# r-barnes/richdem

Hardware: NVIDIA H100
Metric: Priority-Flood fill + D8 flow accumulation throughput (higher is better)
Workload: dtype f32

## Files before the change

richdem_b200/csrc/accum.cu:

```cuda
#include "flowmet.cuh"

#include <cmath>
#include <cooperative_groups.h>
#include <memory>
namespace cg = cooperative_groups;

namespace rdb {

namespace {

constexpr uint32_t kDepsMask = 0xFFu;
constexpr uint32_t kSrcFlag = 0x80000000u;
constexpr int kCodeSole = 32;
constexpr int kCodeSource = 64;
constexpr int kLaneChunk = 1024;

template <bool DINF, class T = float>
__global__ void __launch_bounds__(256) flow_code_kernel(const T *__restrict__ dem, uint8_t *__restrict__ code,
                                                         float *__restrict__ rmaxArr, double *__restrict__ accum,
                                                         int W, int H, T nodata, int ones, int tfilter) {
  const size_t n = (size_t)W * H;
  const size_t i = (size_t)blockIdx.x * blockDim.x + threadIdx.x;
  if (i >= n) return;
  const int y = (int)(i / W), x = (int)(i - (size_t)y * W);
// ... 1364 lines not shown
    k = (int)(wv >> 56);
    sum[x] = (double)(wv & kPkVal);
    cnt[x] = k;
    ghost[x] = 0;
  }
  for (int o = 16; o > 0; o >>= 1) k += __shfl_down_sync(0xffffffffu, k, o);
  if ((threadIdx.x & 31) == 0 && k) atomicAdd(total, k);
}

__global__ void __launch_bounds__(256) band_count_packed_kernel(const unsigned long long *__restrict__ gtop,
                                                                 const unsigned long long *__restrict__ gbot, int W,
                                                                 int *sums) {
  int s0 = 0, s1 = 0;
  for (int x = blockIdx.x * blockDim.x + threadIdx.x; x < W; x += gridDim.x * blockDim.x) {
    if (gtop) s0 += (int)(gtop[x] >> 56);
    if (gbot) s1 += (int)(gbot[x] >> 56);
  }
  for (int o = 16; o > 0; o >>= 1) {
    s0 += __shfl_down_sync(0xffffffffu, s0, o);
    s1 += __shfl_down_sync(0xffffffffu, s1, o);
  }
  if ((threadIdx.x & 31) == 0) {
    if (s0) atomicAdd(&sums[0], s0);
    if (s1) atomicAdd(&sums[1], s1);
  }
}

__global__ void __launch_bounds__(256) band_apply_packed_kernel(unsigned long long *row, const double *__restrict__ sum,
                                                                 const int *__restrict__ cnt, int W, int base_index,
                                                                 int *frontier, int *fcount, double scale) {
  const int x = blockIdx.x * blockDim.x + threadIdx.x;
  if (x >= W) return;
  const int k = cnt[x];
  if (k <= 0) return;
  const unsigned long long wv = row[x];
  const unsigned long long val = (wv & kPkVal) + (unsigned long long)sum[x];
  const unsigned long long left = (wv >> 56) - (unsigned long long)k;
  if (left == 0) {
    row[x] = (unsigned long long)__double_as_longlong((double)val * scale);
    frontier[atomicAdd(fcount, 1)] = base_index + x;
  } else {
    row[x] = (left << 56) | val;
  }
}

constexpr int kFaT = 64;
constexpr int kFaCells = kFaT * kFaT;
constexpr int kFaSlots = 4 * kFaT;
constexpr unsigned long long kLkOne = 1ull << 32;

__device__ __forceinline__ int fa_side(int left) { return left < kFaT ? left : kFaT; }

__device__ __forceinline__ int fa_slot_of(int lx, int ly, int tw, int th) {
  if (ly == 0) return lx;
  if (ly == th - 1) return kFaT + lx;
  if (lx == 0) return 2 * kFaT + ly;
  if (lx == tw - 1) return 3 * kFaT + ly;
  return -1;
}

__device__ __forceinline__ bool fa_slot_cell(int s, int tw, int th, int &lx, int &ly) {
  const int k = s & (kFaT - 1), side = s / kFaT;
  if (side < 2) {
    lx = k;
    ly = side == 0 ? 0 : th - 1;
    return k < tw && (side == 0 || th > 1);
  }
  lx = side == 2 ? 0 : tw - 1;
  ly = k;
  return k > 0 && k < th - 1 && (side == 2 || tw > 1);
}

constexpr int kFaRootExit = 0x8000, kFaRootEnd = 0x4000, kFaRoot = kFaRootExit | kFaRootEnd;

__device__ __forceinline__ int fa_tile_parent(int c, int cd, int tw, int th) {
  const int d = cd & 15;
  if (cd == kCodeNoData || d == 0) return c | kFaRootEnd;
  const int x = (c & (kFaT - 1)) + d8dx(d), y = c / kFaT + d8dy(d);
  if (x < 0 || y < 0 || x >= tw || y >= th) return c | kFaRootExit;
  return y * kFaT + x;
}

template <bool SUM>
__device__ __forceinline__ void fa_tile_jump(uint16_t *sPar, unsigned *sAcc, unsigned live) {
  constexpr int kPer = kFaCells / 256;
  const int t = threadIdx.x;
  while (__syncthreads_or(live)) {
    unsigned pq[kPer], a[kPer];
#pragma unroll
    for (int k = 0; k < kPer; k++) {
      if (live >> k & 1) {
        const int c = t + 256 * k, p = sPar[c], q = sPar[p];
        if (SUM) {
          pq[k] = (unsigned)p | (unsigned)q << 16;
          a[k] = sAcc[c];
        } else {
          sPar[c] = (uint16_t)q;
          if (q & kFaRoot) live &= ~(1u << k);
        }
      }
    }
    if (SUM) {
      __syncthreads();
#pragma unroll
      for (int k = 0; k < kPer; k++) {
        if (live >> k & 1) {
          const int q = pq[k] >> 16;
          atomicAdd(&sAcc[pq[k] & 0xffffu], a[k]);
          sPar[t + 256 * k] = (uint16_t)q;
          if (q & kFaRoot) live &= ~(1u << k);
        }
      }
    }
  }
}

__global__ void __launch_bounds__(256) fa_tile_codes_kernel(const float *__restrict__ dem, uint8_t *__restrict__ code,
                                                             int *__restrict__ link, unsigned long long *__restrict__ lword,
                                                             unsigned *__restrict__ inflow, int W, int H, float nodata,
                                                             int tiles_x) {
  constexpr int kWin = kFaT + 2;
  static_assert(kFaCells * sizeof(uint16_t) <= kWin * kWin * sizeof(float), "the parent array lives in the DEM window");
  __shared__ __align__(16) float sDem[kWin * kWin];
  __shared__ __align__(16) uint8_t sCode[kFaCells];
  __shared__ unsigned sCount[kFaSlots];
  const int t = threadIdx.x, tile = blockIdx.x;
  sCount[t] = 0;
  const int bx = tile % tiles_x, by = tile / tiles_x;
  const int x0 = bx * kFaT, y0 = by * kFaT;
  const int tw = fa_side(W - x0), th = fa_side(H - y0);
  constexpr unsigned kFaNoDataBits = 0x7fffffffu;
  for (int i = t; i < kWin * kWin; i += 256) {
    const int wy = i / kWin, wx = i - wy * kWin;
    const int gy = y0 - 1 + wy, gx = x0 - 1 + wx;
    float v = __uint_as_float(kFaNoDataBits);
    if (gy >= 0 && gy < H && gx >= 0 && gx < W) {
      v = __ldg(dem + (size_t)gy * W + gx);
      v = v == nodata ? __uint_as_float(kFaNoDataBits) : v != v ? __uint_as_float(0x7fc00000u) : v;
    }
    sDem[i] = v;
  }
  __syncthreads();
  {
    const int lx0 = (t & 15) * 4, ly0 = (t >> 4) * 4;
    float a[3][6];
#pragma unroll
    for (int j = 1; j < 3; j++)
#pragma unroll
      for (int k = 0; k < 6; k++) a[j][k] = sDem[(ly0 + j - 1) * kWin + lx0 + k];
#pragma unroll
    for (int j = 0; j < 4; j++) {
      const int ly = ly0 + j, gy = y0 + ly;
#pragma unroll
      for (int k = 0; k < 6; k++) {
        a[0][k] = a[1][k];
        a[1][k] = a[2][k];
        a[2][k] = sDem[(ly + 2) * kWin + lx0 + k];
      }
      unsigned word = 0;
#pragma unroll
      for (int k = 0; k < 4; k++) {
        const int lx = lx0 + k, gx = x0 + lx;
        const float e = a[1][k + 1];
        int cd = 0;
        if (lx >= tw || ly >= th || __float_as_uint(e) == kFaNoDataBits) {
          cd = kCodeNoData;
        } else if (!(gx == 0 || gy == 0 || gx == W - 1 || gy == H - 1)) {
          const float ne[9] = {0.f, a[1][k], a[0][k], a[0][k + 1], a[0][k + 2], a[1][k + 2], a[2][k + 2], a[2][k + 1], a[2][k]};
          float lowest = fminf(e, 3.402823466e+38f);
#pragma unroll
          for (int n = 1; n <= 8; n++) {
            if (ne[n] < lowest) {
              lowest = ne[n];
              cd = n;
            }
          }
        }
        word |= (unsigned)cd << (8 * k);
      }
      *reinterpret_cast<unsigned *>(&sCode[ly * kFaT + lx0]) = word;
    }
  }
  __syncthreads();
  reinterpret_cast<uint4 *>(code + (size_t)tile * kFaCells)[t] = reinterpret_cast<const uint4 *>(sCode)[t];
  uint16_t *sPar = reinterpret_cast<uint16_t *>(sDem);
  unsigned live = 0;
#pragma unroll
  for (int k = 0; k < kFaCells / 256; k++) {
    const int c = t + 256 * k, p = fa_tile_parent(c, sCode[c], tw, th);
    sPar[c] = (uint16_t)p;
    if (!(p & kFaRoot)) live |= 1u << k;
  }
  fa_tile_jump<false>(sPar, nullptr, live);
#pragma unroll
  for (int k = 0; k < kFaCells / 256; k++) {
    const int r = sPar[t + 256 * k];
    if (r & kFaRootExit) atomicAdd(&sCount[fa_slot_of(r & (kFaT - 1), (r & (kFaCells - 1)) / kFaT, tw, th)], 1u);
  }
  __syncthreads();
  const size_t gs = (size_t)tile * kFaSlots + t;
  int lk = -1;
  unsigned long long out = 0;
  int lx, ly;
  if (fa_slot_cell(t, tw, th, lx, ly)) {
    const int c = ly * kFaT + lx, r = sPar[c];
    if (r == (c | kFaRootExit)) {
      const int d = sCode[c] & 15;
      const int gx = x0 + lx + d8dx(d), gy = y0 + ly + d8dy(d), rbx = gx / kFaT, rby = gy / kFaT;
      const int rs = fa_slot_of(gx - rbx * kFaT, gy - rby * kFaT, fa_side(W - rbx * kFaT), fa_side(H - rby * kFaT));
      lk = -2 - ((rby * tiles_x + rbx) * kFaSlots + rs);
      out = kLkOne | sCount[t];
    } else if (r & kFaRootExit) {
      const int e = r & (kFaCells - 1);
      lk = tile * kFaSlots + fa_slot_of(e & (kFaT - 1), e / kFaT, tw, th);
    }
  }
  link[gs] = lk;
  lword[gs] = out;
  inflow[gs] = 0;
}

__device__ __forceinline__ int fa_link_next(const int *link, int r) {
  const int l = link[r];
  return l <= -2 ? r : l;
}

__global__ void __launch_bounds__(256) fa_link_count_kernel(const int *__restrict__ link, unsigned long long *lword,
                                                             int nslots) {
  const int p = blockIdx.x * blockDim.x + threadIdx.x;
  if (p >= nslots) return;
  const int l = link[p];
  if (l > -2) return;
  const int q = fa_link_next(link, -2 - l);
  if (q >= 0) atomicAdd(&lword[q], kLkOne);
}

__global__ void __launch_bounds__(256) fa_link_walk_kernel(const int *__restrict__ link, unsigned long long *lword,
                                                            unsigned *inflow, int nslots) {
  const int p = blockIdx.x * blockDim.x + threadIdx.x;
  if (p >= nslots) return;
  int l = link[p];
  if (l > -2) return;
  const unsigned long long old = atomicAdd(&lword[p], 0ull - kLkOne);
  if ((old >> 32) != 1ull) return;
  unsigned long long acc = old & (kLkOne - 1);
  for (;;) {
    const int r = -2 - l;
    atomicAdd(&inflow[r], (unsigned)acc);
    const int q = fa_link_next(link, r);
    if (q < 0) break;
    const unsigned long long o = atomicAdd(&lword[q], acc - kLkOne);
    if ((o >> 32) != 1ull) break;
    acc = (o & (kLkOne - 1)) + acc;
    l = link[q];
  }
}

__global__ void __launch_bounds__(256) fa_tile_final_kernel(const uint8_t *__restrict__ code,
                                                             const unsigned *__restrict__ inflow, double *__restrict__ accum,
                                                             int W, int H, int tiles_x) {
  constexpr unsigned kNoDataAcc = 0xffffffffu;
  __shared__ __align__(16) unsigned sAcc[kFaCells];
  __shared__ __align__(16) uint16_t sPar[kFaCells];
  __shared__ __align__(16) uint8_t sCode[kFaCells];
  const int t = threadIdx.x, tile = blockIdx.x;
  const int bx = tile % tiles_x, by = tile / tiles_x;
  const int x0 = bx * kFaT, y0 = by * kFaT;
  const int tw = fa_side(W - x0), th = fa_side(H - y0);
  reinterpret_cast<uint4 *>(sCode)[t] = __ldg(reinterpret_cast<const uint4 *>(code + (size_t)tile * kFaCells) + t);
  __syncthreads();
  unsigned live = 0;
#pragma unroll
  for (int k = 0; k < kFaCells / 256; k++) {
    const int c = t + 256 * k, cd = sCode[c], p = fa_tile_parent(c, cd, tw, th);
    sPar[c] = (uint16_t)p;
    sAcc[c] = cd == kCodeNoData ? kNoDataAcc : 1u;
    if (!(p & kFaRoot)) live |= 1u << k;
  }
  __syncthreads();
  int lx, ly;
  if (fa_slot_cell(t, tw, th, lx, ly) && sCode[ly * kFaT + lx] != kCodeNoData)
    sAcc[ly * kFaT + lx] += __ldg(inflow + (size_t)tile * kFaSlots + t);
  fa_tile_jump<true>(sPar, sAcc, live);
  for (int c = 2 * t; c < kFaCells; c += 512) {
    const int cx = c & (kFaT - 1), cy = c / kFaT;
    if (cx >= tw || cy >= th) continue;
    const unsigned s0 = sAcc[c], s1 = sAcc[c + 1];
    const double a0 = s0 == kNoDataAcc ? -1.0 : (double)s0, a1 = s1 == kNoDataAcc ? -1.0 : (double)s1;
    double *out = accum + (size_t)(y0 + cy) * W + x0 + cx;
    if (cx + 1 < tw && ((uintptr_t)out & 15) == 0) {
      *reinterpret_cast<double2 *>(out) = make_double2(a0, a1);
    } else {
      out[0] = a0;
      if (cx + 1 < tw) out[1] = a1;
    }
  }
}

long long fa_tile_slots(int w, int h) {
  return (long long)((w + kFaT - 1) / kFaT) * ((h + kFaT - 1) / kFaT) * kFaSlots;
}

void fa_d8_tiles(const float *d_dem, double *d_accum, int w, int h, float nodata) {
  Ctx &c = ctx();
  const int tiles_x = (w + kFaT - 1) / kFaT;
  const long long nslots = fa_tile_slots(w, h);
  const unsigned ntiles = (unsigned)(nslots / kFaSlots);
  DevBuf<uint8_t> code((size_t)ntiles * kFaCells);
  DevBuf<int> link((size_t)nslots);
  DevBuf<unsigned long long> lword((size_t)nslots);
  DevBuf<unsigned> inflow((size_t)nslots);
  const unsigned sblocks = (unsigned)((nslots + 255) / 256);
  fa_tile_codes_kernel<<<ntiles, 256, 0, c.stream>>>(d_dem, code.p, link.p, lword.p, inflow.p, w, h, nodata, tiles_x);
  fa_link_count_kernel<<<sblocks, 256, 0, c.stream>>>(link.p, lword.p, (int)nslots);
  KernelTimer kt;
  fa_link_walk_kernel<<<sblocks, 256, 0, c.stream>>>(link.p, lword.p, inflow.p, (int)nslots);
  kt.stop_async();
  fa_tile_final_kernel<<<ntiles, 256, 0, c.stream>>>(code.p, inflow.p, d_accum, w, h, tiles_x);
  RDB_CK(cudaGetLastError());
  count_launch(4);
  RDB_CK(cudaStreamSynchronize(c.stream));
  c.stats.ms_main_kernel += kt.ms();
  c.stats.accum_rounds = 1;
}
}

template <class T>
static void fa_fused(const T *d_dem, double *d_accum, int w, int h, T nodata, bool ones, bool dinf) {
  constexpr bool F32 = sizeof(T) == 4;
  Ctx &c = ctx();
  const size_t n = (size_t)w * h;
  if constexpr (F32) {
    if (!dinf && ones && c.params.accum_packed && fa_tile_slots(w, h) < INT32_MAX) {
      fa_d8_tiles(d_dem, d_accum, w, h, nodata);
      return;
    }
  } else if (!dinf) {
    fail("FA_D8 on doubles runs on float keys (fa_fused_dev)");
  }
  DevBuf<uint8_t> code(n);
  DevBuf<float> rmax;
  bool have_codes = false;
  if (dinf && ones && (w & 3) == 0 && ((uintptr_t)d_accum & 15) == 0 && c.params.accum_dinf_packed) {
    rmax.alloc(n);
    const unsigned blocks = (unsigned)((n + 255) / 256);
    unsigned long long *word = reinterpret_cast<unsigned long long *>(d_accum);
    flow_code_kernel<true, T><<<blocks, 256, 0, c.stream>>>(d_dem, code.p, rmax.p, d_accum, w, h, nodata, 1, (int)c.params.flowmet_tarboton_filter);
    have_codes = true;
    DevBuf<DinfShare> share(1);
    RDB_CK(cudaMemsetAsync(share.p, 0, sizeof(DinfShare), c.stream));
    dinf_count_data_kernel<<<c.num_sms * 8, 256, 0, c.stream>>>(code.p, n, share.p);
    RDB_CK(cudaGetLastError());
    count_launch(2);
    DinfShare *hs0 = reinterpret_cast<DinfShare *>(c.pinned);
    RDB_CK(cudaMemcpyAsync(hs0, share.p, sizeof(DinfShare), cudaMemcpyDeviceToHost, c.stream));
    RDB_CK(cudaStreamSynchronize(c.stream));
    const bool use_packed = c.params.accum_dinf_packed == 1 || (long long)hs0->n_noflow * 20 > (long long)hs0->n_data;
    if (use_packed) {
    dim3 blk(256), grd((w / 4 + 255) / 256, h < 8192 ? h : 8192);
    deps_gather_packed_dinf_x4_kernel<<<grd, blk, 0, c.stream>>>(code.p, word, w, h, 0, h);
    RDB_CK(cudaGetLastError());
    count_launch();
    DevBuf<int> list(n);
    DevBuf<unsigned long long> dstats;
    if (c.params.accum_dinf_stats) {
      dstats.alloc(16);
      RDB_CK(cudaMemsetAsync(dstats.p, 0, 16 * sizeof(unsigned long long), c.stream));
    }
    KernelTimer kt;
    launch_walk_dinf(code.p, rmax.p, word, w, (int)n, list.p, share.p, dstats.p, 0, (int)n, -1);
    RDB_CK(cudaGetLastError());
    count_launch(2);
    DinfShare *hs = reinterpret_cast<DinfShare *>(c.pinned);
    RDB_CK(cudaMemcpyAsync(hs, share.p, sizeof(DinfShare), cudaMemcpyDeviceToHost, c.stream));
    kt.stop_async();
    RDB_CK(cudaStreamSynchronize(c.stream));
    c.stats.ms_main_kernel += kt.ms();
    c.stats.accum_rounds = hs->phases;
    if (dstats.p) {
      unsigned long long hsx[16];
      RDB_CK(cudaMemcpy(hsx, dstats.p, sizeof(hsx), cudaMemcpyDeviceToHost));
      fprintf(stderr,
              "[dinf walk] %.2f ms, %llu warps, %d phases: iterations sum %llu max %llu, lane-steps %llu (%.1f %% of the lanes), "
              "hand-overs %llu in the rings, %llu through the list (%llu claimed back)\n",
              kt.ms(), hsx[4], hs->phases, hsx[0], hsx[3], hsx[2], 100.0 * (double)hsx[2] / (32.0 * (double)(hsx[0] ? hsx[0] : 1)),
              hsx[8], hsx[7], hsx[6]);
    }
    if (hs->done != hs->n_data)
      fail("D-infinity accumulation (packed walk): %d of %d cells walked after %d phases", hs->done, hs->n_data, hs->phases);
    return;
    }
  }
  DevBuf<uint32_t> st(n);
  if (dinf && !have_codes) rmax.alloc(n);
  const unsigned blocks = (unsigned)((n + 255) / 256);
  if (have_codes) {
  } else if (dinf)
    flow_code_kernel<true, T><<<blocks, 256, 0, c.stream>>>(d_dem, code.p, rmax.p, d_accum, w, h, nodata, ones ? 1 : 0, (int)c.params.flowmet_tarboton_filter);
  else if constexpr (F32) {
    if ((w & 3) == 0 && ((uintptr_t)d_dem & 15) == 0 && ((uintptr_t)d_accum & 15) == 0) {
      dim3 blk(256), grd((w / 4 + 255) / 256, h < 8192 ? h : 8192);
      flow_code_d8_x4_kernel<<<grd, blk, 0, c.stream>>>(d_dem, code.p, d_accum, w, h, nodata, ones ? 1 : 0);
    } else
      flow_code_kernel<false><<<blocks, 256, 0, c.stream>>>(d_dem, code.p, nullptr, d_accum, w, h, nodata, ones ? 1 : 0, (int)c.params.flowmet_tarboton_filter);
  }
  RDB_CK(cudaGetLastError());
// ... 826 lines not shown
```

richdem_b200/csrc/capi.cu:

```cuda
#include "common.cuh"

#include <algorithm>
#include <cstdlib>
#include <type_traits>

namespace rdb {

static thread_local std::string g_last_error;

void capi_set_error(const char *msg) { g_last_error = msg ? msg : "unknown error"; }

Ctx &ctx() {
  static Ctx c;
  return c;
}

static void init_device(int device) {
  Ctx &c = ctx();
  if (c.inited && c.device == device) return;
  if (c.inited) fail("rdb200_init: already initialised on device %d (call rdb200_shutdown first)", c.device);
  int ndev = 0;
  cudaError_t e = cudaGetDeviceCount(&ndev);
  if (e != cudaSuccess || ndev == 0)
    fail("no CUDA device available (%s); librichdem_b200 has no CPU fallback",
// ... 422 lines not shown

extern "C" {

int rdb200_init(int device) {
  return capi_call([&] { init_device(device); });
}

void rdb200_shutdown(void) {
  Ctx &c = ctx();
  if (!c.inited) return;
  cudaSetDevice(c.device);
  cudaStreamSynchronize(c.stream);
  ws_release_all();
  if (c.pinned) cudaFreeHost(c.pinned);
  cudaEventDestroy(c.ev0);
  cudaEventDestroy(c.ev1);
  cudaEventDestroy(c.evk0);
  cudaEventDestroy(c.evk1);
  cudaStreamDestroy(c.own_stream);
  for (int k = 0; k < 2; k++)
    if (c.aux_stream[k]) cudaStreamDestroy(c.aux_stream[k]);
  for (int k = 0; k < 3; k++)
    if (c.aux_event[k]) cudaEventDestroy(c.aux_event[k]);
  const Params keep = c.params;
  c = Ctx();
  c.params = keep;
}

const char *rdb200_last_error(void) { return g_last_error.c_str(); }
int rdb200_version(void) { return RDB200_VERSION; }

int rdb200_set_stream(void *cuda_stream) {
  return capi_call([&] {
    ensure_init();
    Ctx &c = ctx();
    RDB_CK(cudaStreamSynchronize(c.stream));
    c.stream = cuda_stream ? (cudaStream_t)cuda_stream : c.own_stream;
  });
}

int rdb200_get_stats(rdb200_stats *out) {
  return capi_call([&] {
    if (!out) fail("rdb200_get_stats: null pointer");
    *out = ctx().stats;
  });
}

int rdb200_set_param(const char *name, int64_t value) {
  return capi_call([&] {
    if (!name) fail("rdb200_set_param: null name");
    Params &p = ctx().params;
    const std::string n(name);
    if (n == "reset_defaults") p = Params();
    else if (n == "trim_workspace") {
      if (ctx().inited) {
        RDB_CK(cudaStreamSynchronize(ctx().stream));
        ws_trim();
      }
    }
    else if (n == "fill_max_iters") p.fill_max_iters = value;
    else if (n == "fill_rounds_per_sync") p.fill_rounds_per_sync = value > 0 ? value : 16;
    else if (n == "fill_use_tma") p.fill_use_tma = value;
    else if (n == "fill_external_z") p.fill_external_z = value;
    else if (n == "fill_profile") p.fill_profile = value;
    else if (n == "fill_wake_filter") p.fill_wake_filter = value;
    else if (n == "fill_trace") p.fill_trace = value;
    else if (n == "fill_ordered") p.fill_ordered = value;
    else if (n == "fill_order_rounds") p.fill_order_rounds = value;
    else if (n == "fill_band_rounds") p.fill_band_rounds = value;
    else if (n == "accum_threads") p.accum_threads = value > 0 ? value : 256;
    else if (n == "accum_budget") p.accum_budget = value;
    else if (n == "accum_walk_lanes") p.accum_walk_lanes = value;
    else if (n == "accum_fused_prep") p.accum_fused_prep = value;
    else if (n == "flats_tiled") p.flats_tiled = value;
    else if (n == "flats_pair") p.flats_pair = value;
    else if (n == "flats_fused_classify") p.flats_fused_classify = value;
    else if (n == "fill_multigrid") p.fill_multigrid = value;
    else if (n == "fill_multigrid_min") p.fill_multigrid_min = value;
    else if (n == "fill_vcycle") p.fill_vcycle = value;
    else if (n == "fill_band_multigrid") p.fill_band_multigrid = value;
    else if (n == "flats_uf_tiled") p.flats_uf_tiled = value;
    else if (n == "flowdirs_rolling") p.flowdirs_rolling = value;
    else if (n == "accum_packed") p.accum_packed = value;
    else if (n == "accum_dinf_packed") p.accum_dinf_packed = value;
    else if (n == "accum_dinf_share") p.accum_dinf_share = value;
    else if (n == "flowmet_tarboton_filter") p.flowmet_tarboton_filter = value;
    else if (n == "accum_walk_scan") p.accum_walk_scan = value;
    else if (n == "accum_walk_ahead") p.accum_walk_ahead = value;
    else if (n == "accum_dinf_stats") p.accum_dinf_stats = value;
    else if (n == "accum_dinf_wait") p.accum_dinf_wait = value;
    else if (n == "f64_band_rank_cap") p.f64_band_rank_cap = value;
    else fail("rdb200_set_param: unknown parameter '%s'", name);
  });
}


int rdb200_fill_depressions_d8_f32(float *dem, int32_t w, int32_t h) { return fill_depressions(Side::host, dem, w, h, false); }
int rdb200_fill_depressions_d4_f32(float *dem, int32_t w, int32_t h) { return fill_depressions(Side::host, dem, w, h, true); }
int rdb200_fill_depressions_epsilon_d8_f32(float *dem, int32_t w, int32_t h, float nodata) {
  return fill_depressions_epsilon(Side::host, dem, w, h, nodata, false);
}
int rdb200_fill_depressions_epsilon_d4_f32(float *dem, int32_t w, int32_t h, float nodata) {
  return fill_depressions_epsilon(Side::host, dem, w, h, nodata, true);
}
int rdb200_pit_mask_d8_f32(const float *dem, uint8_t *mask, int32_t w, int32_t h, float nodata) {
  return pit_mask(Side::host, dem, mask, w, h, nodata, false);
}
int rdb200_pit_mask_d4_f32(const float *dem, uint8_t *mask, int32_t w, int32_t h, float nodata) {
  return pit_mask(Side::host, dem, mask, w, h, nodata, true);
}
int rdb200_has_depressions_d8_f32(const float *dem, int32_t w, int32_t h, int32_t *out) {
  return has_depressions(Side::host, dem, w, h, out, false);
}
int rdb200_has_depressions_d4_f32(const float *dem, int32_t w, int32_t h, int32_t *out) {
  return has_depressions(Side::host, dem, w, h, out, true);
}
int rdb200_resolve_flats_epsilon_f32(float *dem, int32_t w, int32_t h, float nodata) {
  return resolve_flats_epsilon(Side::host, dem, w, h, nodata);
}
int rdb200_get_flat_mask_f32(const float *dem, int32_t *flat_mask, int32_t *labels, int32_t w, int32_t h, float nodata) {
  return get_flat_mask(Side::host, dem, flat_mask, labels, w, h, nodata);
}
int rdb200_d8_flow_directions_f32(const float *dem, uint8_t *dirs, int32_t w, int32_t h, float nodata) {
  return d8_flow_directions(Side::host, dem, dirs, w, h, nodata);
}
int rdb200_d8_flow_directions_flats_f32(float *dem, uint8_t *dirs, int32_t w, int32_t h, float nodata, int32_t alter) {
  return d8_flow_directions_flats(Side::host, dem, dirs, w, h, nodata, alter);
}
int rdb200_d8_flow_accum_u8_i32(const uint8_t *dirs, int32_t *area, int32_t w, int32_t h) {
  return d8_flow_accum(Side::host, dirs, area, w, h);
}
int rdb200_fm_d8_f32(const float *dem, float *props, int32_t w, int32_t h, float nodata) {
  return fm(Side::host, 0, dem, props, w, h, nodata);
}
int rdb200_fm_tarboton_f32(const float *dem, float *props, int32_t w, int32_t h, float nodata) {
  return fm(Side::host, 1, dem, props, w, h, nodata);
}
int rdb200_fm_d4_f32(const float *dem, float *props, int32_t w, int32_t h, float nodata) {
  return fm(Side::host, 2, dem, props, w, h, nodata);
}
int rdb200_fm_quinn_f32(const float *dem, float *props, int32_t w, int32_t h, float nodata) {
  return fm(Side::host, 3, dem, props, w, h, nodata, 1.0);
}
int rdb200_fm_holmgren_f32(const float *dem, float *props, int32_t w, int32_t h, float nodata, double xparam) {
  return fm(Side::host, 3, dem, props, w, h, nodata, xparam);
}
int rdb200_fm_freeman_f32(const float *dem, float *props, int32_t w, int32_t h, float nodata, double xparam) {
  return fm(Side::host, 4, dem, props, w, h, nodata, xparam);
}
int rdb200_terrain_attribute_f32(int32_t attribute, const float *dem, float *out, int32_t w, int32_t h, float nodata_in,
                                 float nodata_out, float zscale, double cell_x, double cell_y) {
  return terrain_attribute(Side::host, attribute, dem, out, w, h, nodata_in, nodata_out, zscale, cell_x, cell_y);
}
int rdb200_fa_d4_f32_f64(const float *dem, double *accum, int32_t w, int32_t h, float nodata) {
  return fa_via_props(Side::host, 2, dem, accum, w, h, nodata, 0);
}
int rdb200_fa_quinn_f32_f64(const float *dem, double *accum, int32_t w, int32_t h, float nodata) {
  return fa_via_props(Side::host, 3, dem, accum, w, h, nodata, 1.0);
}
int rdb200_fa_holmgren_f32_f64(const float *dem, double *accum, int32_t w, int32_t h, float nodata, double xparam) {
  return fa_via_props(Side::host, 3, dem, accum, w, h, nodata, xparam);
}
int rdb200_fa_freeman_f32_f64(const float *dem, double *accum, int32_t w, int32_t h, float nodata, double xparam) {
  return fa_via_props(Side::host, 4, dem, accum, w, h, nodata, xparam);
}
int rdb200_flow_accumulation_props_f64(const float *props, double *accum, int32_t w, int32_t h) {
// ... 354 lines not shown
```

richdem_b200/csrc/common.cuh:

```cuda
#pragma once

#include <cuda.h>
#include <cuda_runtime.h>

#include <cstdarg>
#include <cstdint>
#include <cstdio>
#include <cstring>
#include <stdexcept>
#include <string>
#include <vector>

#include "../../include/richdem_b200.h"

struct rdb200_fill_state;

namespace rdb {

struct Error : std::runtime_error {
  using std::runtime_error::runtime_error;
};

[[noreturn]] inline void fail(const char *fmt, ...) {
  char buf[1024];
  va_list ap;
  va_start(ap, fmt);
  vsnprintf(buf, sizeof(buf), fmt, ap);
  va_end(ap);
  throw Error(buf);
}

#define RDB_CK(expr)                                                                        \
  do {                                                                                      \
    cudaError_t _e = (expr);                                                                \
    if (_e != cudaSuccess)                                                                  \
      ::rdb::fail("%s failed at %s:%d: %s", #expr, __FILE__, __LINE__, cudaGetErrorString(_e)); \
  } while (0)

void capi_set_error(const char *msg);

template <class F>
int capi_call(F &&body) {
  try {
    body();
    return 0;
  } catch (const std::exception &e) {
    capi_set_error(e.what());
  } catch (...) {
    capi_set_error("unknown C++ exception");
  }
  return 1;
}

__host__ __device__ __forceinline__ int d8dx(int n) {
  return (int)((0x6a41u >> (2 * n)) & 3u) - 1;
}
__host__ __device__ __forceinline__ int d8dy(int n) {
  return (int)((0x2a405u >> (2 * n)) & 3u) - 1;
}

struct Params {
  int64_t fill_max_iters = 0;
  int64_t fill_rounds_per_sync = 16;
  int64_t fill_use_tma = 1;
  int64_t fill_external_z = 1;
  int64_t fill_ordered = 1;
  int64_t fill_order_rounds = 0;
  int64_t fill_band_rounds = 0;
  int64_t fill_profile = 0;
  int64_t fill_wake_filter = 1;
  int64_t fill_trace = 0;
  int64_t fill_multigrid = 8;
  int64_t fill_vcycle = 8;
  int64_t fill_band_multigrid = 0;
  int64_t fill_multigrid_min = 0;
  int64_t flowdirs_rolling = 1;
  int64_t flats_uf_tiled = 1;
  int64_t flats_fused_classify = 1;
  int64_t flats_pair = 1;
  int64_t flats_tiled = 1;
  int64_t accum_dinf_packed = 1;
  int64_t flowmet_tarboton_filter = 1;
  int64_t accum_walk_ahead = 0;
  int64_t accum_walk_scan = 0;
  int64_t accum_dinf_stats = 0;
  int64_t accum_dinf_share = -1;
  int64_t accum_dinf_wait = 0;
  int64_t accum_packed = 1;
  int64_t accum_fused_prep = 1;
  int64_t accum_walk_lanes = 1;
  int64_t accum_threads = 256;
  int64_t accum_budget = 0;
  int64_t f64_band_rank_cap = 0;
};

struct WsBlock {
  void *ptr;
  size_t bytes;
  bool in_use;
};

struct Ctx {
  bool inited = false;
  int device = -1;
  int num_sms = 0;
  cudaStream_t stream = nullptr;
  cudaStream_t own_stream = nullptr;
  cudaEvent_t ev0 = nullptr, ev1 = nullptr, evk0 = nullptr, evk1 = nullptr;
  cudaStream_t aux_stream[2] = {nullptr, nullptr};
  cudaEvent_t aux_event[3] = {nullptr, nullptr, nullptr};
  std::vector<WsBlock> ws;
  void *pinned = nullptr;
  size_t pinned_bytes = 0;
  rdb200_stats stats;
  Params params;
};

Ctx &ctx();
void ensure_init();
void *ws_alloc(size_t bytes);
void ws_free(void *p);
void ws_release_all();

template <class T>
struct DevBuf {
  T *p = nullptr;
  size_t n = 0;
  DevBuf() = default;
  explicit DevBuf(size_t count) { alloc(count); }
  void alloc(size_t count) {
    reset();
    n = count;
    p = (T *)ws_alloc((count ? count : 1) * sizeof(T));
  }
  void reset() {
    if (p) ws_free(p);
    p = nullptr;
    n = 0;
  }
  ~DevBuf() { reset(); }
  DevBuf(const DevBuf &) = delete;
  DevBuf &operator=(const DevBuf &) = delete;
  operator T *() const { return p; }
};

inline void count_launch(int64_t k = 1) { ctx().stats.kernel_launches += k; }

struct KernelTimer {
  bool active;
  explicit KernelTimer(bool on = true) : active(on) {
    if (active) RDB_CK(cudaEventRecord(ctx().evk0, ctx().stream));
  }
  void stop_async() {
    if (active) RDB_CK(cudaEventRecord(ctx().evk1, ctx().stream));
  }
  double ms() {
    float t = 0;
    if (active) RDB_CK(cudaEventElapsedTime(&t, ctx().evk0, ctx().evk1));
    return t;
  }
};

int comm_rank(const rdb200_comm *c);
int comm_world(const rdb200_comm *c);
void comm_exchange(const rdb200_comm *c, const void *send_up, void *recv_up, const void *send_dn, void *recv_dn, size_t bytes);
void comm_allreduce(const rdb200_comm *c, void *buf, size_t count, int op);
void check_band_args(const char *what, const rdb200_comm *comm, const void *d_band, int w, int hloc, int gt, int gb);
void exchange_band_rows(const rdb200_comm *comm, void *d_band, size_t elem, int w, int hloc, int gt, int gb);
void mgpu_fill_band(const rdb200_comm *comm, float *d_local, int w, int hloc, int gt, int gb, int row0, int H, int *xrounds,
                    bool topo4 = false);
// ... 93 lines not shown
```

Measured before the change: 22370.

## Vectorize tile DEM loads, pad shared window, fold inflow init, add profiling

The tile codes kernel now loads the DEM window with float4 global loads on full, aligned tiles, plus separate halo-column loads, and stores it into a padded shared layout so row reads can use float4. The final kernel stages inflow into shared memory and folds it into accumulator initialisation, removing one block barrier. The codes kernel gains launch_bounds(256,8), which may cap registers. An optional clock64-based per-phase profiler is added behind a new fa_profile parameter, off by default.

```diff
diff --git a/richdem_b200/csrc/accum.cu b/richdem_b200/csrc/accum.cu
--- a/richdem_b200/csrc/accum.cu
+++ b/richdem_b200/csrc/accum.cu
@@ -1470,10 +1470,11 @@
 }
 
 template <bool SUM>
-__device__ __forceinline__ void fa_tile_jump(uint16_t *sPar, unsigned *sAcc, unsigned live) {
+__device__ __forceinline__ int fa_tile_jump(uint16_t *sPar, unsigned *sAcc, unsigned live) {
   constexpr int kPer = kFaCells / 256;
   const int t = threadIdx.x;
-  while (__syncthreads_or(live)) {
+  int rounds = 0;
+  for (; __syncthreads_or(live); rounds++) {
     unsigned pq[kPer], a[kPer];
 #pragma unroll
     for (int k = 0; k < kPer; k++) {
@@ -1501,15 +1502,42 @@
       }
     }
   }
-}
-
-__global__ void __launch_bounds__(256) fa_tile_codes_kernel(const float *__restrict__ dem, uint8_t *__restrict__ code,
+  return rounds;
+}
+
+constexpr int kFpCodesPhases = 5;
+constexpr int kFpFinalPhases = 4;
+constexpr int kFpRounds = 13;
+constexpr int kFpCodes = 0, kFpFinal = kFpCodes + kFpCodesPhases + 1 + kFpRounds;
+constexpr int kFpWords = kFpFinal + kFpFinalPhases + 1 + kFpRounds;
+
+__device__ __forceinline__ long long fa_clock() {
+#ifdef RDB_EMU
+  return 0;
+#else
+  return clock64();
+#endif
+}
+
+template <int NP>
+__device__ __forceinline__ void fa_prof_add(unsigned long long *prof, const long long (&tp)[NP + 1], int rounds) {
+  if (threadIdx.x != 0) return;
+#pragma unroll
+  for (int i = 0; i < NP; i++) atomicAdd(prof + i, (unsigned long long)(tp[i + 1] - tp[i]));
+  atomicAdd(prof + NP, (unsigned long long)(tp[NP] - tp[0]));
+  atomicAdd(prof + NP + 1 + (rounds < kFpRounds ? rounds : kFpRounds - 1), 1ull);
+}
+
+template <bool PROF>
+__global__ void __launch_bounds__(256, 8) fa_tile_codes_kernel(const float *__restrict__ dem, uint8_t *__restrict__ code,
                                                              int *__restrict__ link, unsigned long long *__restrict__ lword,
                                                              unsigned *__restrict__ inflow, int W, int H, float nodata,
-                                                             int tiles_x) {
-  constexpr int kWin = kFaT + 2;
-  static_assert(kFaCells * sizeof(uint16_t) <= kWin * kWin * sizeof(float), "the parent array lives in the DEM window");
-  __shared__ __align__(16) float sDem[kWin * kWin];
+                                                             int tiles_x, unsigned long long *prof) {
+  long long tp[kFpCodesPhases + 1];
+  if constexpr (PROF) tp[0] = fa_clock();
+  constexpr int kWin = kFaT + 2, kWp = kFaT + 8, kWo = 3;
+  static_assert(kFaCells * sizeof(uint16_t) <= kWin * kWp * sizeof(float), "the parent array lives in the DEM window");
+  __shared__ __align__(16) float sDem[kWin * kWp];
   __shared__ __align__(16) uint8_t sCode[kFaCells];
   __shared__ unsigned sCount[kFaSlots];
   const int t = threadIdx.x, tile = blockIdx.x;
@@ -1518,24 +1546,57 @@
   const int x0 = bx * kFaT, y0 = by * kFaT;
   const int tw = fa_side(W - x0), th = fa_side(H - y0);
   constexpr unsigned kFaNoDataBits = 0x7fffffffu;
-  for (int i = t; i < kWin * kWin; i += 256) {
-    const int wy = i / kWin, wx = i - wy * kWin;
-    const int gy = y0 - 1 + wy, gx = x0 - 1 + wx;
-    float v = __uint_as_float(kFaNoDataBits);
-    if (gy >= 0 && gy < H && gx >= 0 && gx < W) {
-      v = __ldg(dem + (size_t)gy * W + gx);
-      v = v == nodata ? __uint_as_float(kFaNoDataBits) : v != v ? __uint_as_float(0x7fc00000u) : v;
-    }
-    sDem[i] = v;
+  const auto canon = [nodata](float v) {
+    return v == nodata ? __uint_as_float(kFaNoDataBits) : v != v ? __uint_as_float(0x7fc00000u) : v;
+  };
+  if (tw == kFaT && (W & 3) == 0 && ((uintptr_t)dem & 15) == 0) {
+    constexpr int kVec = kWin * (kFaT / 4), kVecPer = (kVec + 255) / 256;
+    float4 v[kVecPer];
+#pragma unroll
+    for (int j = 0; j < kVecPer; j++) {
+      const int i = t + 256 * j, gy = y0 - 1 + (i >> 4);
+      v[j] = make_float4(__uint_as_float(kFaNoDataBits), __uint_as_float(kFaNoDataBits), __uint_as_float(kFaNoDataBits),
+                         __uint_as_float(kFaNoDataBits));
+      if (i < kVec && gy >= 0 && gy < H)
+        v[j] = __ldg(reinterpret_cast<const float4 *>(dem + (size_t)gy * W + x0) + (i & 15));
+    }
+    float e = __uint_as_float(kFaNoDataBits);
+    const int ewy = t >> 1, egy = y0 - 1 + ewy, egx = t & 1 ? x0 + kFaT : x0 - 1;
+    if (t < 2 * kWin && egy >= 0 && egy < H && egx >= 0 && egx < W) e = __ldg(dem + (size_t)egy * W + egx);
+#pragma unroll
+    for (int j = 0; j < kVecPer; j++) {
+      const int i = t + 256 * j;
+      if (i < kVec)
+        *reinterpret_cast<float4 *>(&sDem[(i >> 4) * kWp + kWo + 1 + 4 * (i & 15)]) =
+            make_float4(canon(v[j].x), canon(v[j].y), canon(v[j].z), canon(v[j].w));
+    }
+    if (t < 2 * kWin) sDem[ewy * kWp + kWo + (t & 1 ? kWin - 1 : 0)] = canon(e);
+  } else {
+    for (int i = t; i < kWin * kWin; i += 256) {
+      const int wy = i / kWin, wx = i - wy * kWin;
+      const int gy = y0 - 1 + wy, gx = x0 - 1 + wx;
+      float v = __uint_as_float(kFaNoDataBits);
+      if (gy >= 0 && gy < H && gx >= 0 && gx < W) v = canon(__ldg(dem + (size_t)gy * W + gx));
+      sDem[wy * kWp + kWo + wx] = v;
+    }
   }
   __syncthreads();
+  if constexpr (PROF) tp[1] = fa_clock();
   {
     const int lx0 = (t & 15) * 4, ly0 = (t >> 4) * 4;
     float a[3][6];
-#pragma unroll
-    for (int j = 1; j < 3; j++)
-#pragma unroll
-      for (int k = 0; k < 6; k++) a[j][k] = sDem[(ly0 + j - 1) * kWin + lx0 + k];
+    const auto load_row = [&](float(&r)[6], int wy) {
+      const float *row = sDem + wy * kWp + kWo + lx0;
+      const float4 m = *reinterpret_cast<const float4 *>(row + 1);
+      r[0] = row[0];
+      r[1] = m.x;
+      r[2] = m.y;
+      r[3] = m.z;
+      r[4] = m.w;
+      r[5] = row[5];
+    };
+    load_row(a[1], ly0);
+    load_row(a[2], ly0 + 1);
 #pragma unroll
     for (int j = 0; j < 4; j++) {
       const int ly = ly0 + j, gy = y0 + ly;
@@ -1543,8 +1604,8 @@
       for (int k = 0; k < 6; k++) {
         a[0][k] = a[1][k];
         a[1][k] = a[2][k];
-        a[2][k] = sDem[(ly + 2) * kWin + lx0 + k];
-      }
+      }
+      load_row(a[2], ly + 2);
       unsigned word = 0;
 #pragma unroll
       for (int k = 0; k < 4; k++) {
@@ -1570,6 +1631,7 @@
     }
   }
   __syncthreads();
+  if constexpr (PROF) tp[2] = fa_clock();
   reinterpret_cast<uint4 *>(code + (size_t)tile * kFaCells)[t] = reinterpret_cast<const uint4 *>(sCode)[t];
   uint16_t *sPar = reinterpret_cast<uint16_t *>(sDem);
   unsigned live = 0;
@@ -1579,13 +1641,15 @@
     sPar[c] = (uint16_t)p;
     if (!(p & kFaRoot)) live |= 1u << k;
   }
-  fa_tile_jump<false>(sPar, nullptr, live);
+  const int rounds = fa_tile_jump<false>(sPar, nullptr, live);
+  if constexpr (PROF) tp[3] = fa_clock();
 #pragma unroll
   for (int k = 0; k < kFaCells / 256; k++) {
     const int r = sPar[t + 256 * k];
     if (r & kFaRootExit) atomicAdd(&sCount[fa_slot_of(r & (kFaT - 1), (r & (kFaCells - 1)) / kFaT, tw, th)], 1u);
   }
   __syncthreads();
+  if constexpr (PROF) tp[4] = fa_clock();
   const size_t gs = (size_t)tile * kFaSlots + t;
   int lk = -1;
   unsigned long long out = 0;
@@ -1606,6 +1670,11 @@
   link[gs] = lk;
   lword[gs] = out;
   inflow[gs] = 0;
+  if constexpr (PROF) {
+    __syncthreads();
+    tp[5] = fa_clock();
+    fa_prof_add<kFpCodesPhases>(prof + kFpCodes, tp, rounds);
+  }
 }
 
 __device__ __forceinline__ int fa_link_next(const int *link, int r) {
@@ -1644,32 +1713,40 @@
   }
 }
 
+template <bool PROF>
 __global__ void __launch_bounds__(256) fa_tile_final_kernel(const uint8_t *__restrict__ code,
                                                              const unsigned *__restrict__ inflow, double *__restrict__ accum,
-                                                             int W, int H, int tiles_x) {
+                                                             int W, int H, int tiles_x, unsigned long long *prof) {
+  long long tp[kFpFinalPhases + 1];
+  if constexpr (PROF) tp[0] = fa_clock();
   constexpr unsigned kNoDataAcc = 0xffffffffu;
   __shared__ __align__(16) unsigned sAcc[kFaCells];
   __shared__ __align__(16) uint16_t sPar[kFaCells];
   __shared__ __align__(16) uint8_t sCode[kFaCells];
+  __shared__ unsigned sIn[kFaSlots];
   const int t = threadIdx.x, tile = blockIdx.x;
   const int bx = tile % tiles_x, by = tile / tiles_x;
   const int x0 = bx * kFaT, y0 = by * kFaT;
   const int tw = fa_side(W - x0), th = fa_side(H - y0);
   reinterpret_cast<uint4 *>(sCode)[t] = __ldg(reinterpret_cast<const uint4 *>(code + (size_t)tile * kFaCells) + t);
+  sIn[t] = __ldg(inflow + (size_t)tile * kFaSlots + t);
   __syncthreads();
+  if constexpr (PROF) tp[1] = fa_clock();
   unsigned live = 0;
 #pragma unroll
   for (int k = 0; k < kFaCells / 256; k++) {
     const int c = t + 256 * k, cd = sCode[c], p = fa_tile_parent(c, cd, tw, th);
+    const int s = fa_slot_of(c & (kFaT - 1), c / kFaT, tw, th);
     sPar[c] = (uint16_t)p;
-    sAcc[c] = cd == kCodeNoData ? kNoDataAcc : 1u;
+    sAcc[c] = cd == kCodeNoData ? kNoDataAcc : 1u + (s >= 0 ? sIn[s] : 0u);
     if (!(p & kFaRoot)) live |= 1u << k;
   }
-  __syncthreads();
-  int lx, ly;
-  if (fa_slot_cell(t, tw, th, lx, ly) && sCode[ly * kFaT + lx] != kCodeNoData)
-    sAcc[ly * kFaT + lx] += __ldg(inflow + (size_t)tile * kFaSlots + t);
-  fa_tile_jump<true>(sPar, sAcc, live);
+  if constexpr (PROF) {
+    __syncthreads();
+    tp[2] = fa_clock();
+  }
+  const int rounds = fa_tile_jump<true>(sPar, sAcc, live);
+  if constexpr (PROF) tp[3] = fa_clock();
   for (int c = 2 * t; c < kFaCells; c += 512) {
     const int cx = c & (kFaT - 1), cy = c / kFaT;
     if (cx >= tw || cy >= th) continue;
@@ -1683,10 +1760,42 @@
       if (cx + 1 < tw) out[1] = a1;
     }
   }
+  if constexpr (PROF) {
+    __syncthreads();
+    tp[4] = fa_clock();
+    fa_prof_add<kFpFinalPhases>(prof + kFpFinal, tp, rounds);
+  }
 }
 
 long long fa_tile_slots(int w, int h) {
   return (long long)((w + kFaT - 1) / kFaT) * ((h + kFaT - 1) / kFaT) * kFaSlots;
+}
+
+void fa_profile_report(const unsigned long long *d_prof, cudaEvent_t (&ev)[4], unsigned ntiles) {
+  unsigned long long h[kFpWords];
+  RDB_CK(cudaMemcpy(h, d_prof, sizeof(h), cudaMemcpyDeviceToHost));
+  int res_codes = 0, res_final = 0;
+  RDB_CK(cudaOccupancyMaxActiveBlocksPerMultiprocessor(&res_codes, fa_tile_codes_kernel<true>, 256, 0));
+  RDB_CK(cudaOccupancyMaxActiveBlocksPerMultiprocessor(&res_final, fa_tile_final_kernel<true>, 256, 0));
+  float ms[2];
+  RDB_CK(cudaEventElapsedTime(&ms[0], ev[0], ev[1]));
+  RDB_CK(cudaEventElapsedTime(&ms[1], ev[2], ev[3]));
+  for (cudaEvent_t e : ev) RDB_CK(cudaEventDestroy(e));
+  struct {
+    const char *pass;
+    int base, nphases, resident;
+    const char *names[kFpCodesPhases];
+  } passes[2] = {{"codes", kFpCodes, kFpCodesPhases, res_codes, {"load", "codes", "jump", "exits", "slots"}},
+                 {"final", kFpFinal, kFpFinalPhases, res_final, {"load", "init", "jump", "write", nullptr}}};
+  for (int p = 0; p < 2; p++) {
+    const auto &q = passes[p];
+    fprintf(stderr, "[fa profile] pass=%s ms=%.4f ctas=%u sms=%d resident=%d cycles=%llu", q.pass, ms[p], ntiles,
+            ctx().num_sms, q.resident, h[q.base + q.nphases]);
+    for (int i = 0; i < q.nphases; i++) fprintf(stderr, " %s=%llu", q.names[i], h[q.base + i]);
+    fprintf(stderr, " rounds=");
+    for (int i = 0; i < kFpRounds; i++) fprintf(stderr, "%llu%s", h[q.base + q.nphases + 1 + i], i + 1 < kFpRounds ? "," : "");
+    fprintf(stderr, "\n");
+  }
 }
 
 void fa_d8_tiles(const float *d_dem, double *d_accum, int w, int h, float nodata) {
@@ -1699,17 +1808,37 @@
   DevBuf<unsigned long long> lword((size_t)nslots);
   DevBuf<unsigned> inflow((size_t)nslots);
   const unsigned sblocks = (unsigned)((nslots + 255) / 256);
-  fa_tile_codes_kernel<<<ntiles, 256, 0, c.stream>>>(d_dem, code.p, link.p, lword.p, inflow.p, w, h, nodata, tiles_x);
+  const bool profile = c.params.fa_profile != 0;
+  DevBuf<unsigned long long> prof(profile ? kFpWords : 0);
+  cudaEvent_t ev[4] = {};
+  if (profile) {
+    RDB_CK(cudaMemsetAsync(prof.p, 0, kFpWords * sizeof(unsigned long long), c.stream));
+    for (cudaEvent_t &e : ev) RDB_CK(cudaEventCreate(&e));
+    RDB_CK(cudaEventRecord(ev[0], c.stream));
+    fa_tile_codes_kernel<true><<<ntiles, 256, 0, c.stream>>>(d_dem, code.p, link.p, lword.p, inflow.p, w, h, nodata, tiles_x,
+                                                             prof.p);
+    RDB_CK(cudaEventRecord(ev[1], c.stream));
+  } else {
+    fa_tile_codes_kernel<false><<<ntiles, 256, 0, c.stream>>>(d_dem, code.p, link.p, lword.p, inflow.p, w, h, nodata, tiles_x,
+                                                              nullptr);
+  }
   fa_link_count_kernel<<<sblocks, 256, 0, c.stream>>>(link.p, lword.p, (int)nslots);
   KernelTimer kt;
   fa_link_walk_kernel<<<sblocks, 256, 0, c.stream>>>(link.p, lword.p, inflow.p, (int)nslots);
   kt.stop_async();
-  fa_tile_final_kernel<<<ntiles, 256, 0, c.stream>>>(code.p, inflow.p, d_accum, w, h, tiles_x);
+  if (profile) {
+    RDB_CK(cudaEventRecord(ev[2], c.stream));
+    fa_tile_final_kernel<true><<<ntiles, 256, 0, c.stream>>>(code.p, inflow.p, d_accum, w, h, tiles_x, prof.p);
+    RDB_CK(cudaEventRecord(ev[3], c.stream));
+  } else {
+    fa_tile_final_kernel<false><<<ntiles, 256, 0, c.stream>>>(code.p, inflow.p, d_accum, w, h, tiles_x, nullptr);
+  }
   RDB_CK(cudaGetLastError());
   count_launch(4);
   RDB_CK(cudaStreamSynchronize(c.stream));
   c.stats.ms_main_kernel += kt.ms();
   c.stats.accum_rounds = 1;
+  if (profile) fa_profile_report(prof.p, ev, ntiles);
 }
 }
 
diff --git a/richdem_b200/csrc/capi.cu b/richdem_b200/csrc/capi.cu
--- a/richdem_b200/csrc/capi.cu
+++ b/richdem_b200/csrc/capi.cu
@@ -528,6 +528,7 @@
     else if (n == "flats_uf_tiled") p.flats_uf_tiled = value;
     else if (n == "flowdirs_rolling") p.flowdirs_rolling = value;
     else if (n == "accum_packed") p.accum_packed = value;
+    else if (n == "fa_profile") p.fa_profile = value;
     else if (n == "accum_dinf_packed") p.accum_dinf_packed = value;
     else if (n == "accum_dinf_share") p.accum_dinf_share = value;
     else if (n == "flowmet_tarboton_filter") p.flowmet_tarboton_filter = value;
diff --git a/richdem_b200/csrc/common.cuh b/richdem_b200/csrc/common.cuh
--- a/richdem_b200/csrc/common.cuh
+++ b/richdem_b200/csrc/common.cuh
@@ -86,6 +86,7 @@
   int64_t accum_dinf_stats = 0;
   int64_t accum_dinf_share = -1;
   int64_t accum_dinf_wait = 0;
+  int64_t fa_profile = 0;
   int64_t accum_packed = 1;
   int64_t accum_fused_prep = 1;
   int64_t accum_walk_lanes = 1;
```

Result: no change. 22500, median of 6 (+0.6%).
